# robot-learning-freiburg/CL-SLAM

Hardware: AMD Instinct MI355X
Metric: online-adapt frames/sec @192x640 (1 triplet + K replay) (higher is better)
Workload: dtype f32; 1 GPU; DepthPosePrediction.adapt(steps=1), 192x640, 1 online + K=4 replay triplets (global batch 5); ResNet-18 depth+pose nets, closed-form random-init weights; a frame = 5 triplets (value = steps/s * B/5); global_batch=5, replay_k=4, height=192, width=640, adapt_steps_per_frame=1, parallelism=single, lcd_encoder_in_frame=False

## Files before the change

cl-slam_amd/csrc/wgrad_patch.hip:

```cpp
#include "common.h"

namespace clslam {

struct WgPatchK {
    const float* __restrict__ dz;
    const float* __restrict__ src_a;
    const float* __restrict__ src_b;
    float* __restrict__ partial;
    int B, Hi, Wi, Ca, Cb, Ho, Wo, Cout;
    int pad, pad_mode, ups;
    int tilesX, tilesY, ntiles, tiles_per_split, co_tiles, ci_tiles;
};

template <int TH, int TW, int COT, int CIT>
__global__ __launch_bounds__(256) void conv3x3_wgrad_patch_kernel(WgPatchK p) {
    constexpr int BM = TH * TW;
    constexpr int PH = TH + 2, PW = TW + 2, PP = PH * PW;
    constexpr int LDZ = (COT % 32 == 16) ? COT : COT + 16;
    constexpr int LDP = (CIT % 32 == 16) ? CIT : CIT + 16;
    constexpr int TI = COT / 16, TJ = CIT / 16;
    constexpr int Z_F4 = BM * COT / 4, P_F4 = PP * CIT / 4;
    constexpr int Z_IT = (Z_F4 + 255) / 256, P_IT = (P_F4 + 255) / 256;

    constexpr int SMEM = (BM * LDZ + PP * LDP) > (4 * TI * TJ * 256) ? (BM * LDZ + PP * LDP) : (4 * TI * TJ * 256);
    __shared__ __attribute__((aligned(16))) float smem[SMEM];
    float* const Zs = smem;
    float* const Ps = smem + BM * LDZ;

    const int tid = threadIdx.x, lane = tid & 63, wave = tid >> 6;
    const int cot = blockIdx.x % p.co_tiles, cit = blockIdx.x / p.co_tiles;
    const int split = blockIdx.y;
    const int co0 = cot * COT, ci0 = cit * CIT;
    const int Cin = p.Ca + p.Cb;
    const int HA = p.ups ? (p.Hi >> 1) : p.Hi, WA = p.ups ? (p.Wi >> 1) : p.Wi;
    const bool fromA = ci0 < p.Ca;
    const int csrc = fromA ? ci0 : ci0 - p.Ca;
    const int Csrc = fromA ? p.Ca : p.Cb;

    static_assert(TW % 4 == 0, "a pixel quad must not straddle two tile rows");
    const float* __restrict__ src = fromA ? p.src_a : p.src_b;
    f32x4 acc[9][TI][TJ];
#pragma unroll
    for (int t = 0; t < 9; ++t)
#pragma unroll
        for (int i = 0; i < TI; ++i)
#pragma unroll
            for (int j = 0; j < TJ; ++j)
#pragma unroll
                for (int r = 0; r < 4; ++r) acc[t][i][j][r] = 0.f;

    const int l16 = lane & 15, kg = lane >> 4;
    const int t_beg = split * p.tiles_per_split;
    const int t_end = min(p.ntiles, t_beg + p.tiles_per_split);

    float4 rz[Z_IT], rp[P_IT];
    bool okz[Z_IT], okp[P_IT];
    auto load_tile = [&](int tile) {
        int q = tile;
        const int tx = q % p.tilesX; q /= p.tilesX;
        const int ty = q % p.tilesY; q /= p.tilesY;
        const int b = q;
        const int oy0 = ty * TH, ox0 = tx * TW;
#pragma unroll
        for (int it = 0; it < Z_IT; ++it) {
            const int f = tid + it * 256;
            const int m = f / (COT / 4), c4 = f % (COT / 4);
            const int oy = oy0 + m / TW, ox = ox0 + m % TW;
            const bool ok = (f < Z_F4) && oy < p.Ho && ox < p.Wo;
            const size_t o = ok ? (((size_t)b * p.Ho + oy) * p.Wo + ox) * p.Cout + co0 + c4 * 4 : 0;
            rz[it] = *reinterpret_cast<const float4*>(p.dz + o);
            okz[it] = ok;
        }
#pragma unroll
        for (int it = 0; it < P_IT; ++it) {
            const int f = tid + it * 256;
            const int pp = f / (CIT / 4), c4 = f % (CIT / 4);
            const int pr = pp / PW, pc = pp - pr * PW;
            int iy = oy0 - p.pad + pr, ix = ox0 - p.pad + pc;
            bool ok = f < P_F4;
            if (p.pad_mode == CLSLAM_PAD_REFLECT) {
                iy = reflect_idx(iy, p.Hi); ix = reflect_idx(ix, p.Wi);
                iy = min(max(iy, 0), p.Hi - 1); ix = min(max(ix, 0), p.Wi - 1);
            } else {
                ok = ok && iy >= 0 && iy < p.Hi && ix >= 0 && ix < p.Wi;
            }
            size_t o = 0;
            if (ok) {
                if (fromA) {
                    const int sy = p.ups ? (iy >> 1) : iy, sx = p.ups ? (ix >> 1) : ix;
                    o = ((size_t)(b * HA + sy) * WA + sx) * Csrc + csrc + c4 * 4;
                } else {
                    o = ((size_t)(b * p.Hi + iy) * p.Wi + ix) * Csrc + csrc + c4 * 4;
                }
            }
            rp[it] = *reinterpret_cast<const float4*>(src + o);
            okp[it] = ok;
        }
    };
    auto store_tile = [&]() {
#pragma unroll
        for (int it = 0; it < Z_IT; ++it) {
            const int f = tid + it * 256;
            float4 v = rz[it];
            if (!okz[it]) v = make_float4(0.f, 0.f, 0.f, 0.f);
            if (f < Z_F4) *reinterpret_cast<float4*>(&Zs[(f / (COT / 4)) * LDZ + (f % (COT / 4)) * 4]) = v;
        }
#pragma unroll
        for (int it = 0; it < P_IT; ++it) {
            const int f = tid + it * 256;
            float4 v = rp[it];
            if (!okp[it]) v = make_float4(0.f, 0.f, 0.f, 0.f);
            if (f < P_F4) *reinterpret_cast<float4*>(&Ps[(f / (CIT / 4)) * LDP + (f % (CIT / 4)) * 4]) = v;
        }
    };

    if (t_beg < t_end) load_tile(t_beg);
    for (int tile = t_beg; tile < t_end; ++tile) {
        __syncthreads();
        store_tile();
        __syncthreads();
        if (tile + 1 < t_end) load_tile(tile + 1);
#pragma unroll 2
        for (int ks = wave; ks < BM / 4; ks += 4) {
            const int pix = ks * 4 + kg;
            const int prow = (pix / TW) * PW + (pix % TW);
            float a[TI];
#pragma unroll
            for (int i = 0; i < TI; ++i) a[i] = Zs[pix * LDZ + i * 16 + l16];
#pragma unroll
            for (int tap = 0; tap < 9; ++tap) {
                const int off = (tap / 3) * PW + (tap % 3);
#pragma unroll
                for (int j = 0; j < TJ; ++j) {
                    const float bv = Ps[(prow + off) * LDP + j * 16 + l16];
#pragma unroll
                    for (int i = 0; i < TI; ++i) acc[tap][i][j] = mfma_16x16x4(a[i], bv, acc[tap][i][j]);
                }
            }
        }
    }

    float* out = p.partial + (size_t)split * p.Cout * 9 * Cin;
    float* red = smem;
#pragma unroll
    for (int tap = 0; tap < 9; ++tap) {
        __syncthreads();
#pragma unroll
        for (int i = 0; i < TI; ++i)
#pragma unroll
            for (int j = 0; j < TJ; ++j)
                *reinterpret_cast<f32x4*>(&red[((wave * TI * TJ + i * TJ + j) * 64 + lane) * 4]) = acc[tap][i][j];
        __syncthreads();
        for (int e = tid; e < TI * TJ * 64; e += 256) {
            const int ij = e / 64, ln = e % 64;
            f32x4 s4 = *reinterpret_cast<const f32x4*>(&red[(ij * 64 + ln) * 4]);
#pragma unroll
            for (int w = 1; w < 4; ++w) {
                const f32x4 v = *reinterpret_cast<const f32x4*>(&red[((w * TI * TJ + ij) * 64 + ln) * 4]);
                s4 += v;
            }
            const int i = ij / TJ, j = ij % TJ;
            const int ci = ci0 + j * 16 + (ln & 15);
#pragma unroll
            for (int r = 0; r < 4; ++r) {
                const int co = co0 + i * 16 + 4 * (ln >> 4) + r;
                out[((size_t)co * 9 + tap) * Cin + ci] = s4[r];
            }
        }
    }
}

template <int TH, int TW, int COT, int CIT>
static int launch_wgp(WgPatchK k, int splits, hipStream_t stream) {
    k.co_tiles = k.Cout / COT;
    k.ci_tiles = (k.Ca + k.Cb) / CIT;
    hipLaunchKernelGGL((conv3x3_wgrad_patch_kernel<TH, TW, COT, CIT>), dim3(k.co_tiles * k.ci_tiles, splits), dim3(256), 0,
                       stream, k);
    return check_launch("conv3x3_wgrad_patch");
}

static void wgp_tile(const clslam_conv_desc* d, int* cot, int* cit) {
    const int Cin = d->ch_a + d->ch_b;
    const bool c32 = d->ch_out % 32 == 0;
    const bool i32 = Cin % 32 == 0 && (d->ch_b == 0 || d->ch_a % 32 == 0);
    *cot = c32 ? 32 : 16;
    *cit = i32 ? 32 : 16;
    if (*cot == 32 && *cit == 16) *cot = 16;
}

static void wgp_pixel_tile(const clslam_conv_desc* d, int* th, int* tw) {
    int cot, cit;
    wgp_tile(d, &cot, &cit);
    *th = 8; *tw = 16;
    const char* env = getenv("CLSLAM_WGRAD_DEEP_TILES");
    const bool deep = env && atoi(env) != 0;
    if (cot == 32 && cit == 32 && deep) {
        if (d->out_w == 40 && d->out_h % 4 == 0) { *th = 4; *tw = 40; }
        else if (d->out_w == 20 && d->out_h == 6) { *th = 6; *tw = 20; }
    }
}

}

using namespace clslam;

extern "C" int clslam_wgrad_patch_supported(const clslam_conv_desc* d) {
    if (!(d->ksize == 3 && d->stride == 1 && d->out_h == d->in_h + 2 * d->pad - 2 && d->out_w == d->in_w + 2 * d->pad - 2 &&
          d->ch_out % 16 == 0 && (d->ch_a + d->ch_b) % 16 == 0 && d->ch_a % 16 == 0))
        return 0;
    if (d->out_w > 40) return 1;
    int th, tw;
    wgp_pixel_tile(d, &th, &tw);
    return th != 8;
}

extern "C" int clslam_wgrad_patch_splits(const clslam_conv_desc* d, int target_blocks) {
    int cot, cit, th, tw;
    wgp_tile(d, &cot, &cit);
    wgp_pixel_tile(d, &th, &tw);
    const int cols = (d->ch_out / cot) * ((d->ch_a + d->ch_b) / cit);
    const int ntiles = d->batch * cdiv(d->out_h, th) * cdiv(d->out_w, tw);
    const int splits = std::max(1, std::min(ntiles, cdiv(target_blocks, cols)));
    const int tps = cdiv(ntiles, splits);
    return cdiv(ntiles, tps);
}

extern "C" int clslam_conv_wgrad_patch(const clslam_conv_desc* d, const float* dz, float* partial, int splits, void* stream_) {
    hipStream_t stream = (hipStream_t)stream_;
    CLSLAM_REQUIRE(d && dz && partial && splits >= 1 && clslam_wgrad_patch_supported(d), "conv_wgrad_patch: unsupported conv");
    int cot, cit, th, tw;
    wgp_tile(d, &cot, &cit);
    wgp_pixel_tile(d, &th, &tw);
    WgPatchK k;
    k.dz = dz; k.src_a = d->src_a; k.src_b = d->src_b; k.partial = partial;
    k.B = d->batch; k.Hi = d->in_h; k.Wi = d->in_w; k.Ca = d->ch_a; k.Cb = d->ch_b; k.Ho = d->out_h; k.Wo = d->out_w;
    k.Cout = d->ch_out; k.pad = d->pad; k.pad_mode = d->pad_mode; k.ups = d->upsample_a;
    k.tilesX = cdiv(k.Wo, tw); k.tilesY = cdiv(k.Ho, th);
    k.ntiles = k.B * k.tilesX * k.tilesY;
    k.tiles_per_split = cdiv(k.ntiles, splits);
    k.co_tiles = k.ci_tiles = 0;
    if (th == 4) return launch_wgp<4, 40, 32, 32>(k, splits, stream);
    if (th == 6) return launch_wgp<6, 20, 32, 32>(k, splits, stream);
    if (cot == 32) return launch_wgp<8, 16, 32, 32>(k, splits, stream);
    if (cit == 32) return launch_wgp<8, 16, 16, 32>(k, splits, stream);
    return launch_wgp<8, 16, 16, 16>(k, splits, stream);
}
```

Before: 354.1 frames/s.

## Split wgrad taps across grid groups and enable deep tiles by default

```diff
diff --git a/cl-slam_amd/csrc/wgrad_patch.hip b/cl-slam_amd/csrc/wgrad_patch.hip
--- a/cl-slam_amd/csrc/wgrad_patch.hip
+++ b/cl-slam_amd/csrc/wgrad_patch.hip
@@ -12,10 +12,12 @@
     int tilesX, tilesY, ntiles, tiles_per_split, co_tiles, ci_tiles;
 };
 
-template <int TH, int TW, int COT, int CIT>
+template <int TH, int TW, int COT, int CIT, int NG>
 __global__ __launch_bounds__(256) void conv3x3_wgrad_patch_kernel(WgPatchK p) {
+    static_assert(NG == 1 || NG == 2 || NG == 3, "tap groups: 9, 5+4 or 3+3+3");
+    constexpr int NT = (9 + NG - 1) / NG;
     constexpr int BM = TH * TW;
-    constexpr int PH = TH + 2, PW = TW + 2, PP = PH * PW;
+    constexpr int PH = (NG == 3) ? TH : TH + 2, PW = TW + 2, PP = PH * PW;
     constexpr int LDZ = (COT % 32 == 16) ? COT : COT + 16;
     constexpr int LDP = (CIT % 32 == 16) ? CIT : CIT + 16;
     constexpr int TI = COT / 16, TJ = CIT / 16;
@@ -30,6 +32,10 @@
     const int tid = threadIdx.x, lane = tid & 63, wave = tid >> 6;
     const int cot = blockIdx.x % p.co_tiles, cit = blockIdx.x / p.co_tiles;
     const int split = blockIdx.y;
+    const int grp = (NG == 1) ? 0 : (int)blockIdx.z;
+    const int tap0 = grp * NT;
+    const int ntap = min(NT, 9 - tap0);
+    const int prow0 = (NG == 3) ? grp : 0;
     const int co0 = cot * COT, ci0 = cit * CIT;
     const int Cin = p.Ca + p.Cb;
     const int HA = p.ups ? (p.Hi >> 1) : p.Hi, WA = p.ups ? (p.Wi >> 1) : p.Wi;
@@ -39,9 +45,9 @@
 
     static_assert(TW % 4 == 0, "a pixel quad must not straddle two tile rows");
     const float* __restrict__ src = fromA ? p.src_a : p.src_b;
-    f32x4 acc[9][TI][TJ];
-#pragma unroll
-    for (int t = 0; t < 9; ++t)
+    f32x4 acc[NT][TI][TJ];
+#pragma unroll
+    for (int t = 0; t < NT; ++t)
 #pragma unroll
         for (int i = 0; i < TI; ++i)
 #pragma unroll
@@ -76,7 +82,7 @@
             const int f = tid + it * 256;
             const int pp = f / (CIT / 4), c4 = f % (CIT / 4);
             const int pr = pp / PW, pc = pp - pr * PW;
-            int iy = oy0 - p.pad + pr, ix = ox0 - p.pad + pc;
+            int iy = oy0 - p.pad + prow0 + pr, ix = ox0 - p.pad + pc;
             bool ok = f < P_F4;
             if (p.pad_mode == CLSLAM_PAD_REFLECT) {
                 iy = reflect_idx(iy, p.Hi); ix = reflect_idx(ix, p.Wi);
@@ -128,13 +134,15 @@
 #pragma unroll
             for (int i = 0; i < TI; ++i) a[i] = Zs[pix * LDZ + i * 16 + l16];
 #pragma unroll
-            for (int tap = 0; tap < 9; ++tap) {
-                const int off = (tap / 3) * PW + (tap % 3);
+            for (int t = 0; t < NT; ++t) {
+                if (NG == 2 && t >= ntap) continue;
+                const int tap = tap0 + t;
+                const int off = (NG == 3) ? t : (tap / 3) * PW + (tap % 3);
 #pragma unroll
                 for (int j = 0; j < TJ; ++j) {
                     const float bv = Ps[(prow + off) * LDP + j * 16 + l16];
 #pragma unroll
-                    for (int i = 0; i < TI; ++i) acc[tap][i][j] = mfma_16x16x4(a[i], bv, acc[tap][i][j]);
+                    for (int i = 0; i < TI; ++i) acc[t][i][j] = mfma_16x16x4(a[i], bv, acc[t][i][j]);
                 }
             }
         }
@@ -143,13 +151,15 @@
     float* out = p.partial + (size_t)split * p.Cout * 9 * Cin;
     float* red = smem;
 #pragma unroll
-    for (int tap = 0; tap < 9; ++tap) {
+    for (int t = 0; t < NT; ++t) {
+        if (t >= ntap) break;
+        const int tap = tap0 + t;
         __syncthreads();
 #pragma unroll
         for (int i = 0; i < TI; ++i)
 #pragma unroll
             for (int j = 0; j < TJ; ++j)
-                *reinterpret_cast<f32x4*>(&red[((wave * TI * TJ + i * TJ + j) * 64 + lane) * 4]) = acc[tap][i][j];
+                *reinterpret_cast<f32x4*>(&red[((wave * TI * TJ + i * TJ + j) * 64 + lane) * 4]) = acc[t][i][j];
         __syncthreads();
         for (int e = tid; e < TI * TJ * 64; e += 256) {
             const int ij = e / 64, ln = e % 64;
@@ -170,56 +180,106 @@
     }
 }
 
-template <int TH, int TW, int COT, int CIT>
+template <int TH, int TW, int COT, int CIT, int NG>
 static int launch_wgp(WgPatchK k, int splits, hipStream_t stream) {
     k.co_tiles = k.Cout / COT;
     k.ci_tiles = (k.Ca + k.Cb) / CIT;
-    hipLaunchKernelGGL((conv3x3_wgrad_patch_kernel<TH, TW, COT, CIT>), dim3(k.co_tiles * k.ci_tiles, splits), dim3(256), 0,
-                       stream, k);
+    hipLaunchKernelGGL((conv3x3_wgrad_patch_kernel<TH, TW, COT, CIT, NG>), dim3(k.co_tiles * k.ci_tiles, splits, NG), dim3(256),
+                       0, stream, k);
     return check_launch("conv3x3_wgrad_patch");
 }
 
-static void wgp_tile(const clslam_conv_desc* d, int* cot, int* cit) {
+struct WgPlan {
+    int th, tw, cot, cit, ng;
+};
+
+struct WgVariant {
+    WgPlan v;
+    int (*launch)(WgPatchK, int, hipStream_t);
+};
+
+#define WGP_VARIANT(TH, TW, COT, CIT, NG) {{TH, TW, COT, CIT, NG}, &launch_wgp<TH, TW, COT, CIT, NG>}
+static const WgVariant kWgVariants[] = {
+    WGP_VARIANT(8, 16, 16, 16, 1), WGP_VARIANT(8, 16, 16, 32, 1), WGP_VARIANT(8, 16, 32, 32, 1),
+    WGP_VARIANT(4, 40, 32, 32, 1), WGP_VARIANT(6, 20, 32, 32, 1),
+    WGP_VARIANT(8, 16, 32, 32, 2), WGP_VARIANT(8, 16, 32, 32, 3), WGP_VARIANT(4, 16, 32, 32, 3),
+    WGP_VARIANT(4, 16, 64, 32, 3),
+    WGP_VARIANT(4, 40, 32, 32, 3), WGP_VARIANT(2, 40, 32, 32, 3), WGP_VARIANT(6, 20, 32, 32, 3),
+};
+#undef WGP_VARIANT
+
+static const WgVariant* wgp_find(const WgPlan& q) {
+    for (const WgVariant& e : kWgVariants)
+        if (e.v.th == q.th && e.v.tw == q.tw && e.v.cot == q.cot && e.v.cit == q.cit && e.v.ng == q.ng) return &e;
+    return nullptr;
+}
+
+static bool wgp_channels_ok(const clslam_conv_desc* d, int cot, int cit) {
     const int Cin = d->ch_a + d->ch_b;
-    const bool c32 = d->ch_out % 32 == 0;
-    const bool i32 = Cin % 32 == 0 && (d->ch_b == 0 || d->ch_a % 32 == 0);
-    *cot = c32 ? 32 : 16;
-    *cit = i32 ? 32 : 16;
-    if (*cot == 32 && *cit == 16) *cot = 16;
-}
-
-static void wgp_pixel_tile(const clslam_conv_desc* d, int* th, int* tw) {
-    int cot, cit;
-    wgp_tile(d, &cot, &cit);
-    *th = 8; *tw = 16;
-    const char* env = getenv("CLSLAM_WGRAD_DEEP_TILES");
-    const bool deep = env && atoi(env) != 0;
-    if (cot == 32 && cit == 32 && deep) {
-        if (d->out_w == 40 && d->out_h % 4 == 0) { *th = 4; *tw = 40; }
-        else if (d->out_w == 20 && d->out_h == 6) { *th = 6; *tw = 20; }
-    }
-}
-
-}
-
-using namespace clslam;
-
-extern "C" int clslam_wgrad_patch_supported(const clslam_conv_desc* d) {
+    return d->ch_out % cot == 0 && Cin % cit == 0 && (d->ch_b == 0 || d->ch_a % cit == 0);
+}
+
+static bool env_pair(const char* name, int* a, int* b) {
+    const char* e = getenv(name);
+    return e && sscanf(e, "%dx%d", a, b) == 2;
+}
+
+static bool env_list_has(const char* name, int v) {
+    const char* e = getenv(name);
+    if (!e) return true;
+    for (const char* c = e; *c;) {
+        if (atoi(c) == v) return true;
+        while (*c && *c != ',') ++c;
+        if (*c == ',') ++c;
+    }
+    return false;
+}
+
+constexpr int WGP_DEEP_DEFAULT = 3;
+
+static bool wgp_plan(const clslam_conv_desc* d, WgPlan* out) {
     if (!(d->ksize == 3 && d->stride == 1 && d->out_h == d->in_h + 2 * d->pad - 2 && d->out_w == d->in_w + 2 * d->pad - 2 &&
           d->ch_out % 16 == 0 && (d->ch_a + d->ch_b) % 16 == 0 && d->ch_a % 16 == 0))
-        return 0;
-    if (d->out_w > 40) return 1;
-    int th, tw;
-    wgp_pixel_tile(d, &th, &tw);
-    return th != 8;
+        return false;
+    WgPlan pl;
+    pl.cot = 16; pl.cit = wgp_channels_ok(d, 16, 32) ? 32 : 16;
+    if (wgp_channels_ok(d, 32, 32)) pl.cot = 32;
+    pl.th = 8; pl.tw = 16; pl.ng = 1;
+    bool have = d->out_w > 40;
+    const char* env = getenv("CLSLAM_WGRAD_DEEP_TILES");
+    const int deep = env ? atoi(env) : WGP_DEEP_DEFAULT;
+    if (pl.cot == 32 && pl.cit == 32 && deep != 0) {
+        const bool s40 = d->out_w == 40 && d->out_h % 4 == 0, s20 = d->out_w == 20 && d->out_h == 6;
+        if (s40) { pl.th = deep == 3 ? 2 : 4; pl.tw = 40; have = true; }
+        else if (s20) { pl.th = 6; pl.tw = 20; have = true; }
+        if (have && deep >= 2) pl.ng = 3;
+    }
+    if (env_list_has("CLSLAM_WGRAD_PLAN_W", d->out_w)) {
+        WgPlan q = pl;
+        bool any = env_pair("CLSLAM_WGRAD_CTILE", &q.cot, &q.cit);
+        any = env_pair("CLSLAM_WGRAD_PTILE", &q.th, &q.tw) || any;
+        const char* g = getenv("CLSLAM_WGRAD_TAPGROUPS");
+        if (g) { q.ng = atoi(g); any = true; }
+        if (any && q.cot > 0 && q.cit > 0 && wgp_channels_ok(d, q.cot, q.cit) && wgp_find(q)) { pl = q; have = true; }
+    }
+    *out = pl;
+    return have;
+}
+
+}
+
+using namespace clslam;
+
+extern "C" int clslam_wgrad_patch_supported(const clslam_conv_desc* d) {
+    WgPlan pl;
+    return wgp_plan(d, &pl) ? 1 : 0;
 }
 
 extern "C" int clslam_wgrad_patch_splits(const clslam_conv_desc* d, int target_blocks) {
-    int cot, cit, th, tw;
-    wgp_tile(d, &cot, &cit);
-    wgp_pixel_tile(d, &th, &tw);
-    const int cols = (d->ch_out / cot) * ((d->ch_a + d->ch_b) / cit);
-    const int ntiles = d->batch * cdiv(d->out_h, th) * cdiv(d->out_w, tw);
+    WgPlan pl;
+    wgp_plan(d, &pl);
+    const int cols = (d->ch_out / pl.cot) * ((d->ch_a + d->ch_b) / pl.cit) * pl.ng;
+    const int ntiles = d->batch * cdiv(d->out_h, pl.th) * cdiv(d->out_w, pl.tw);
     const int splits = std::max(1, std::min(ntiles, cdiv(target_blocks, cols)));
     const int tps = cdiv(ntiles, splits);
     return cdiv(ntiles, tps);
@@ -227,21 +287,17 @@
 
 extern "C" int clslam_conv_wgrad_patch(const clslam_conv_desc* d, const float* dz, float* partial, int splits, void* stream_) {
     hipStream_t stream = (hipStream_t)stream_;
-    CLSLAM_REQUIRE(d && dz && partial && splits >= 1 && clslam_wgrad_patch_supported(d), "conv_wgrad_patch: unsupported conv");
-    int cot, cit, th, tw;
-    wgp_tile(d, &cot, &cit);
-    wgp_pixel_tile(d, &th, &tw);
+    WgPlan pl;
+    CLSLAM_REQUIRE(d && dz && partial && splits >= 1 && wgp_plan(d, &pl), "conv_wgrad_patch: unsupported conv");
+    const WgVariant* var = wgp_find(pl);
+    CLSLAM_REQUIRE(var, "conv_wgrad_patch: no kernel for the layer's plan");
     WgPatchK k;
     k.dz = dz; k.src_a = d->src_a; k.src_b = d->src_b; k.partial = partial;
     k.B = d->batch; k.Hi = d->in_h; k.Wi = d->in_w; k.Ca = d->ch_a; k.Cb = d->ch_b; k.Ho = d->out_h; k.Wo = d->out_w;
     k.Cout = d->ch_out; k.pad = d->pad; k.pad_mode = d->pad_mode; k.ups = d->upsample_a;
-    k.tilesX = cdiv(k.Wo, tw); k.tilesY = cdiv(k.Ho, th);
+    k.tilesX = cdiv(k.Wo, pl.tw); k.tilesY = cdiv(k.Ho, pl.th);
     k.ntiles = k.B * k.tilesX * k.tilesY;
     k.tiles_per_split = cdiv(k.ntiles, splits);
     k.co_tiles = k.ci_tiles = 0;
-    if (th == 4) return launch_wgp<4, 40, 32, 32>(k, splits, stream);
-    if (th == 6) return launch_wgp<6, 20, 32, 32>(k, splits, stream);
-    if (cot == 32) return launch_wgp<8, 16, 32, 32>(k, splits, stream);
-    if (cit == 32) return launch_wgp<8, 16, 16, 32>(k, splits, stream);
-    return launch_wgp<8, 16, 16, 16>(k, splits, stream);
-}
+    return var->launch(k, splits, stream);
+}
```

Result: no change. 354.1 frames/s, median of 4 (+0.0%).
